# robotsorcerer/LevelSetPy

Hardware: AMD Instinct MI355X
Metric: grid-cell RK-substep updates/sec, Dubins-3D HJI 201^3 fp64 (higher is better)
Workload: dtype f64

## Files before the change

### levelsetpy_amd/csrc/hj_device.h

```cpp
#pragma once
#ifndef __HIPCC_RTC__
#include <hip/hip_runtime.h>
#endif
#include "../../include/hj_mi355x.h"

namespace hj {

template <typename T> struct Lim;
template <> struct Lim<double> { static constexpr double tiny = 1e-99; static constexpr double lowest = -1.0e300; };
template <> struct Lim<float>  { static constexpr float  tiny = 1e-30f; static constexpr float lowest = -3.0e38f; };

template <typename T> __device__ __forceinline__ T weno_eps_uncontracted(T max_d1sq) {
#pragma clang fp contract(off)
    const T a = T(1e-6) * max_d1sq;
    return a + Lim<T>::tiny;
}

template <typename T> __device__ __forceinline__ T t_abs(T x) { return x < T(0) ? -x : x; }
template <> __device__ __forceinline__ double t_abs<double>(double x) { return __builtin_fabs(x); }
template <> __device__ __forceinline__ float  t_abs<float>(float x)   { return __builtin_fabsf(x); }

__device__ __forceinline__ double max_acc(double a, double b) {
    double r;
    asm("v_max_f64 %0, %1, %2" : "=v"(r) : "v"(a), "v"(b));
// ... 268 lines not shown
        pc = T(45) * D1 + (T(-9) * D2 + D3);
        hd = T(15) * S1 + (T(-6) * S2 + (S3 + T(-20) * v[3]));
    } else if constexpr (SCHEME == HJ_WENO5) {
        const WenoLine<T> ln = weno5_line(v);
        T lq[3], rq[3];
        weno5_left_q(ln, wk, lq);
        weno5_right_q(ln, wk, rq);
        weno5_combine(ln, lq, rq, pc, hd);
    } else if constexpr ((SCHEME == HJ_ENO3 || SCHEME == HJ_ENO2) && HJ_ENO_EXACT) {
#pragma clang fp contract(off)
        DD<T> t;
        dd_tables(v, K, t);
        const T dx = K[3], dx2 = K[4], tdx2 = K[5];
        const bool sL0 = t_abs(t.D2[1]) < t_abs(t.D2[2]), sL1 = t_abs(t.D2[2]) < t_abs(t.D2[3]);
        T L, R;
        if constexpr (SCHEME == HJ_ENO2) {
            const T eL = dx * (sL0 ? t.D2[1] : t.D2[2]);
            const T eR = dx * (sL1 ? t.D2[2] : t.D2[3]);
            L = t.D1[2] + eL;
            R = t.D1[3] - eR;
        } else {
            const bool sT0 = t_abs(t.D3[0]) < t_abs(t.D3[1]), sT1 = t_abs(t.D3[1]) < t_abs(t.D3[2]);
            const bool sT2 = t_abs(t.D3[2]) < t_abs(t.D3[3]);
            const bool lRR = !sL0 && !sT1;
            const T l2 = dx * (lRR ? t.D2[2] : t.D2[1]);
            const T l3a = tdx2 * ((sL0 && sT0) ? t.D3[0] : t.D3[1]);
            const T l3b = dx2 * t.D3[2];
            const T lb = t.D1[2] + l2;
            L = lRR ? (lb - l3b) : (lb + l3a);
            const bool rRR = !sL1 && !sT2;
            const T r2 = dx * (rRR ? t.D2[3] : t.D2[2]);
            const T r3a = dx2 * ((sL1 && sT1) ? t.D3[1] : t.D3[2]);
            const T r3b = tdx2 * t.D3[3];
            const T rb = t.D1[3] - r2;
            R = rRR ? (rb + r3b) : (rb - r3a);
        }
        pc = T(0.5) * (L + R);
        hd = T(0.5) * (R - L);
    } else if constexpr (base_scheme(SCHEME) == HJ_ENO3) {
        const T u0 = v[1] - v[0], u1 = v[2] - v[1], u2 = v[3] - v[2];
        const T u3 = v[4] - v[3], u4 = v[5] - v[4], u5 = v[6] - v[5];
        const T s0 = u1 - u0, s1 = u2 - u1, s2 = u3 - u2, s3 = u4 - u3, s4 = u5 - u4;
        const T t0 = s1 - s0, t1 = s2 - s1, t2 = s3 - s2, t3 = s4 - s3;
        const bool sL0 = t_abs(s1) < t_abs(s2), sL1 = t_abs(s2) < t_abs(s3);
        const bool sT0 = t_abs(t0) < t_abs(t1), sT1 = t_abs(t1) < t_abs(t2), sT2 = t_abs(t2) < t_abs(t3);
        const T third = T(1) / T(3), sixth = T(1) / T(6);
        const T h1 = T(0.5) * s1, h2 = T(0.5) * s2, h3 = T(0.5) * s3;
        const T qL0 = third * t0 + h1, qL1 = third * t1 + h1, qL2 = h2 - sixth * t2;
        const T qR0 = -sixth * t1 - h2, qR1 = -sixth * t2 - h2, qR2 = third * t3 - h3;
        const T Lq = u2 + (sL0 ? (sT0 ? qL0 : qL1) : (sT1 ? qL1 : qL2));
        const T Rq = u3 + (sL1 ? (sT1 ? qR0 : qR1) : (sT2 ? qR1 : qR2));
        pc = Lq + Rq;
        hd = Rq - Lq;
    } else if constexpr (base_scheme(SCHEME) == HJ_ENO2) {
        const T u1 = v[2] - v[1], u2 = v[3] - v[2], u3 = v[4] - v[3], u4 = v[5] - v[4];
        const T s1 = u2 - u1, s2 = u3 - u2, s3 = u4 - u3;
        const T Lq = u2 + T(0.5) * ((t_abs(s1) < t_abs(s2)) ? s1 : s2);
        const T Rq = u3 + T(-0.5) * ((t_abs(s2) < t_abs(s3)) ? s2 : s3);
        pc = Lq + Rq;
        hd = Rq - Lq;
    } else {
        T L, R;
        upwind<SCHEME, T>(v, K, eps, L, R);
        pc = T(0.5) * (L + R);
        hd = T(0.5) * (R - L);
    }
}

#ifndef HJ_PAR_SLOTS
#define HJ_PAR_SLOTS 8
#endif
template <typename T> struct HamTables {
    const T* coord[HJ_MAX_DIM];
    const T* aux[4];
    T par[HJ_PAR_SLOTS];
    const unsigned long long* range;
    int local_mode;
};
__device__ __forceinline__ double key_value(unsigned long long k) {
    const unsigned long long b = (k & 0x8000000000000000ull) ? (k & 0x7fffffffffffffffull) : ~k;
    return __longlong_as_double((long long)b);
}

template <typename T> struct HamDubinsRel {
    static constexpr int ND = 3;
    static constexpr int ID = HJ_HAM_DUBINS_REL;
    static constexpr unsigned PLANE_DEP = 0x2;
    struct Cell { T a, b, x1, alpha0; };
    struct Plane { T x0, awx0; };
    struct Raw { T c, s, x1; };
    __device__ static __forceinline__ Raw cell_raw(const HamTables<T>& P, const int* idx) {
        return Raw{P.aux[0][idx[2]], P.aux[1][idx[2]], P.coord[1][idx[1]]};
    }
    __device__ static __forceinline__ Raw cell_raw_next(const HamTables<T>& P, const int* idx, const Raw& first) {
        return Raw{P.aux[0][idx[2]], P.aux[1][idx[2]], first.x1};
    }
    __device__ static __forceinline__ Cell cell_fin(const HamTables<T>& P, const Raw& r, const T* sc) {
#pragma clang fp contract(off)
        Cell c;
        const T a = P.par[0] - P.par[1] * r.c;
        const T b = P.par[1] * r.s;
        const T x1 = r.x1;
        c.alpha0 = sc[0] * (t_abs(a) + t_abs(P.par[2] * x1));
        c.a = sc[0] * a;
        c.b = sc[1] * b;
        c.x1 = sc[0] * x1;
        return c;
    }
    __device__ static __forceinline__ Cell cell(const HamTables<T>& P, const int* idx, const T* sc) {
        return cell_fin(P, cell_raw(P, idx), sc);
    }
    __device__ static __forceinline__ Plane plane(const HamTables<T>& P, int i0, const T* sc) {
        Plane u;
        const T x0 = P.coord[0][i0];
        u.x0 = sc[1] * x0;
        u.awx0 = sc[1] * t_abs(P.par[2] * x0);
        return u;
    }
    template <bool NP = false>
    __device__ static __forceinline__ void eval(const HamTables<T>& P, const Cell& c, const Plane& u,
                                                const T* sc, const T* q, T& H, T* alpha) {
        const T w = P.par[2];
        const T p2 = sc[2] * q[2];
        if constexpr (NP) {
#pragma clang fp contract(off)
            H = q[0] * c.a - q[1] * c.b - w * t_abs(q[0] * c.x1 - q[1] * u.x0 - p2) + w * t_abs(p2);
        } else {
            H = q[0] * c.a - q[1] * c.b - w * t_abs(q[0] * c.x1 - q[1] * u.x0 - p2) + w * t_abs(p2);
        }
        alpha[0] = c.alpha0;
        alpha[1] = t_abs(c.b) + u.awx0;
        alpha[2] = sc[2] * P.par[3];
    }
};

template <typename T> struct HamDoubleIntegrator {
    static constexpr int ND = 2;
    static constexpr int ID = HJ_HAM_DOUBLE_INTEGRATOR;
    static constexpr unsigned PLANE_DEP = 0x0;
    struct Cell { T x1, alpha0; };
    struct Plane { int unused; };
    struct Raw { T x1; };
    __device__ static __forceinline__ Raw cell_raw(const HamTables<T>& P, const int* idx) { return Raw{P.coord[1][idx[1]]}; }
    __device__ static __forceinline__ Raw cell_raw_next(const HamTables<T>& P, const int* idx, const Raw&) { return cell_raw(P, idx); }
    __device__ static __forceinline__ Cell cell_fin(const HamTables<T>&, const Raw& r, const T* sc) {
        Cell c;
        c.x1 = sc[0] * r.x1;
        c.alpha0 = sc[0] * t_abs(r.x1);
        return c;
    }
    __device__ static __forceinline__ Cell cell(const HamTables<T>& P, const int* idx, const T* sc) {
        return cell_fin(P, cell_raw(P, idx), sc);
    }
    __device__ static __forceinline__ Plane plane(const HamTables<T>&, int, const T*) { return Plane{0}; }
    template <bool NP = false>
    __device__ static __forceinline__ void eval(const HamTables<T>& P, const Cell& c, const Plane&,
                                                const T* sc, const T* q, T& H, T* alpha) {
        const T us = sc[1] * P.par[0];
        if constexpr (NP) {
#pragma clang fp contract(off)
            H = -(q[0] * c.x1 - t_abs(q[1]) * us);
        } else {
            H = -(q[0] * c.x1 - t_abs(q[1]) * us);
        }
        alpha[0] = c.alpha0;
        alpha[1] = t_abs(us);
    }
};

template <typename T> struct HamDoublePendulum {
    static constexpr int ND = 4;
    static constexpr int ID = HJ_HAM_DOUBLE_PENDULUM;
    static constexpr unsigned PLANE_DEP = 0xA;
    struct Cell { T w1, w2, s2, c2; };
    struct Plane { T s1, c1; };
    using Raw = Cell;
    struct Row { T a1, b1, c1, a3, b3, c3; };
    struct TCell { T w1s, w1q, w2s, w2q; };
    static constexpr int ROW_AXIS = 2;
    __device__ static __forceinline__ Row row(T s1, T c1, T s2, T c2, const T* sc) {
        const T G = T(9.8);
        const T sd = s2 * c1 - c2 * s1;
        const T cd = c2 * c1 + s2 * s1;
        const T den = T(2) - cd * cd;
        const T rden = T(1) / den;
        const T a = (sd * cd) * rden, c = sd * rden;
        const T b1 = (G * (s2 * cd - T(2) * s1)) * rden;
        const T b3 = (T(2) * G * (s1 * cd - s2)) * rden;
        Row r;
        r.a1 = sc[1] * a; r.b1 = sc[1] * b1; r.c1 = sc[1] * c;
        r.a3 = -(sc[3] * a); r.b3 = sc[3] * b3; r.c3 = T(-2) * (sc[3] * c);
        return r;
    }
    __device__ static __forceinline__ Row row_at(const HamTables<T>& P, int i0, int irow, const T* sc) {
        return row(P.aux[0][i0], P.aux[1][i0], P.aux[2][irow], P.aux[3][irow], sc);
    }
    __device__ static __forceinline__ TCell tcell(const Cell& c, const T* sc) {
        return TCell{sc[0] * c.w1, c.w1 * c.w1, sc[2] * c.w2, c.w2 * c.w2};
    }
    __device__ static __forceinline__ void eval_row(const HamTables<T>& P, const TCell& c, const Row& r, const T* sc, const T* q, T& H, T* alpha) {
        const T us1 = sc[1] * P.par[0], us3 = sc[3] * P.par[0];
        const T f1s = r.a1 * c.w1q + (r.c1 * c.w2q + r.b1);
        const T f3s = r.a3 * c.w2q + (r.c3 * c.w1q + r.b3);
        H = q[0] * c.w1s + (q[1] * f1s + (q[2] * c.w2s + (q[3] * f3s + (us1 * t_abs(q[1]) + us3 * t_abs(q[3])))));
        alpha[0] = t_abs(c.w1s);
        alpha[1] = t_abs(f1s) + us1;
        alpha[2] = t_abs(c.w2s);
        alpha[3] = t_abs(f3s) + us3;
    }
    __device__ static __forceinline__ Raw cell_raw(const HamTables<T>& P, const int* idx) {
        Cell c;
        c.w1 = P.coord[1][idx[1]];
        c.w2 = P.coord[3][idx[3]];
        c.s2 = P.aux[2][idx[2]];
        c.c2 = P.aux[3][idx[2]];
        return c;
    }
    __device__ static __forceinline__ Raw cell_raw_next(const HamTables<T>& P, const int* idx, const Raw& first) {
        Cell c = first;
        c.w2 = P.coord[3][idx[3]];
        return c;
    }
    __device__ static __forceinline__ Cell cell_fin(const HamTables<T>&, const Raw& r, const T*) { return r; }
    __device__ static __forceinline__ Cell cell(const HamTables<T>& P, const int* idx, const T* sc) {
        return cell_fin(P, cell_raw(P, idx), sc);
    }
    __device__ static __forceinline__ Plane plane(const HamTables<T>& P, int i0, const T*) {
        Plane u;
        u.s1 = P.aux[0][i0];
        u.c1 = P.aux[1][i0];
        return u;
    }
    template <bool NP = false>
    __device__ static __forceinline__ void eval(const HamTables<T>& P, const Cell& c, const Plane& pl,
                                                const T* sc, const T* q, T& H, T* alpha) {
        eval_row(P, tcell(c, sc), row(pl.s1, pl.c1, c.s2, c.c2, sc), sc, q, H, alpha);
    }
};
template <typename...> struct hj_void { typedef void type; };
template <typename H, typename = void> struct ham_xp { static constexpr bool value = false; };
template <typename H> struct ham_xp<H, typename hj_void<decltype(H::XPOSED)>::type> { static constexpr bool value = H::XPOSED; };
template <typename H> __host__ __device__ constexpr int ham_gaxis(int k) { return ham_xp<H>::value ? (k == 0 ? 1 : (k == 1 ? 0 : k)) : k; }

template <typename T> struct HamDubinsRelX {
    static constexpr int ND = 3;
    static constexpr int ID = HJ_HAM_DUBINS_REL;
    static constexpr bool XPOSED = true;
    static constexpr unsigned PLANE_DEP = 0x2;
    struct Cell { T a, b, x0, absa, alpha1; };
    struct Plane { T x1, awx1; };
    struct Raw { T c, s, x0; };
    __device__ static __forceinline__ Raw cell_raw(const HamTables<T>& P, const int* idx) {
        return Raw{P.aux[0][idx[2]], P.aux[1][idx[2]], P.coord[0][idx[1]]};
    }
    __device__ static __forceinline__ Raw cell_raw_next(const HamTables<T>& P, const int* idx, const Raw& first) {
        return Raw{P.aux[0][idx[2]], P.aux[1][idx[2]], first.x0};
    }
    __device__ static __forceinline__ Cell cell_fin(const HamTables<T>& P, const Raw& r, const T* sc) {
#pragma clang fp contract(off)
        Cell c;
        const T a = P.par[0] - P.par[1] * r.c;
        const T b = P.par[1] * r.s;
        c.absa = t_abs(a);
        c.a = sc[1] * a;
        c.b = sc[0] * b;
        c.x0 = sc[0] * r.x0;
        const T wx0 = P.par[2] * r.x0;
        const T awx0 = sc[0] * t_abs(wx0);
        c.alpha1 = t_abs(c.b) + awx0;
        return c;
    }
    __device__ static __forceinline__ Cell cell(const HamTables<T>& P, const int* idx, const T* sc) {
        return cell_fin(P, cell_raw(P, idx), sc);
    }
    __device__ static __forceinline__ Plane plane(const HamTables<T>& P, int im, const T* sc) {
#pragma clang fp contract(off)
        Plane u;
        const T x1 = P.coord[1][im];
        u.x1 = sc[1] * x1;
        const T wx1 = P.par[2] * x1;
        u.awx1 = t_abs(wx1);
        return u;
    }
    template <bool NP = false>
    __device__ static __forceinline__ void eval(const HamTables<T>& P, const Cell& c, const Plane& u,
                                                const T* sc, const T* q, T& H, T* alpha) {
        const T w = P.par[2];
        const T p2 = sc[2] * q[2];
        if constexpr (NP) {
#pragma clang fp contract(off)
            H = q[1] * c.a - q[0] * c.b - w * t_abs(q[1] * u.x1 - q[0] * c.x0 - p2) + w * t_abs(p2);
        } else {
            H = q[1] * c.a - q[0] * c.b - w * t_abs(q[1] * u.x1 - q[0] * c.x0 - p2) + w * t_abs(p2);
        }
        {
#pragma clang fp contract(off)
            const T sum = c.absa + u.awx1;
            alpha[1] = sc[1] * sum;
        }
        alpha[0] = c.alpha1;
        alpha[2] = sc[2] * P.par[3];
    }
};

template <typename H, typename = void> struct ham_has_rows { static constexpr bool value = false; };
template <typename H> struct ham_has_rows<H, typename hj_void<typename H::Row>::type> { static constexpr bool value = true; };

template <typename H, typename = void> struct ham_reads_range { static constexpr bool value = false; };
template <typename H> struct ham_reads_range<H, typename hj_void<decltype(H::RANGE)>::type> { static constexpr bool value = H::RANGE; };

template <bool NP, typename HAM, typename T>
__device__ __forceinline__ void lf_eval_local(const HamTables<T>& P, const typename HAM::Cell& c, const typename HAM::Plane& u,
                                              const T* sc, const T* pc, const T* hd, T& H, T* alpha) {
    constexpr int ND = HAM::ND;
    T lo[ND], hi[ND];
#pragma unroll
    for (int d = 0; d < ND; ++d) {
        const T a = sc[d] * (pc[d] - hd[d]), b = sc[d] * (pc[d] + hd[d]);
        lo[d] = a < b ? a : b;
        hi[d] = a < b ? b : a;
    }
    if (P.local_mode == 2) {
        typename HAM::Plane v = u;
#pragma unroll
        for (int d = 0; d < ND; ++d) { v.dmin[d] = lo[d]; v.dmax[d] = hi[d]; }
        HAM::template eval<NP>(P, c, v, sc, pc, H, alpha);
    } else {
#pragma unroll
        for (int i = 0; i < ND; ++i) {
            typename HAM::Plane v = u;
            v.dmin[i] = lo[i]; v.dmax[i] = hi[i];
            T Hi, ai[ND];
            HAM::template eval<NP>(P, c, v, sc, pc, Hi, ai);
            alpha[i] = ai[i];
            if (i == 0) H = Hi;
        }
    }
}

template <bool NP, typename HAM, typename T>
__device__ __forceinline__ T lf_ydot(const HamTables<T>& P, const typename HAM::Cell& c, const typename HAM::Plane& u,
                                     const T* sc, const T* pc, const T* hd, T* alpha) {
    T H;
    if constexpr (ham_reads_range<HAM>::value) {
        if (P.local_mode != 0) lf_eval_local<NP, HAM>(P, c, u, sc, pc, hd, H, alpha);
        else HAM::template eval<NP>(P, c, u, sc, pc, H, alpha);
    } else {
        HAM::template eval<NP>(P, c, u, sc, pc, H, alpha);
    }
    if constexpr (NP) {
#pragma clang fp contract(off)
        T diss = T(0);
#pragma unroll
        for (int g = 0; g < HAM::ND; ++g) diss = diss + hd[ham_gaxis<HAM>(g)] * alpha[ham_gaxis<HAM>(g)];
        return -(H - diss);
    } else {
        T diss = T(0);
#pragma unroll
        for (int g = 0; g < HAM::ND; ++g) diss += hd[ham_gaxis<HAM>(g)] * alpha[ham_gaxis<HAM>(g)];
        return -(H - diss);
    }
// ... 90 lines not shown
```

### levelsetpy_amd/csrc/hj_fusedv.h

```cpp
#pragma once
#include "hj_fused.h"

namespace hj {

#if (defined(HJ_ST_UNSAFE) || defined(HJ_ABLATE_NOSYNC) || defined(HJ_ABLATE)) && !defined(HJ_TUNE_BUILD)
#error "HJ_ST_UNSAFE / HJ_ABLATE* give wrong results: tuning builds (-DHJ_TUNE_BUILD) only"
#endif

template <typename T> struct Pair;
template <> struct Pair<double> { typedef double V __attribute__((ext_vector_type(2))); };
template <> struct Pair<float> { typedef float V __attribute__((ext_vector_type(2))); };

#ifndef HJ_PAIR_AUX_Y0
#define HJ_PAIR_AUX_Y0 0
#endif
#ifndef HJ_PAIR_AUX_OUT
#define HJ_PAIR_AUX_OUT 0
#endif
template <int AUX = 0>
__device__ __forceinline__ Pair<double>::V buf_load2(__amdgpu_buffer_rsrc_t r, unsigned off, unsigned soff, double) {
    return __builtin_bit_cast(Pair<double>::V, __builtin_amdgcn_raw_buffer_load_b128(r, off, soff, AUX));
}
template <int AUX = 0>
__device__ __forceinline__ Pair<float>::V buf_load2(__amdgpu_buffer_rsrc_t r, unsigned off, unsigned soff, float) {
    return __builtin_bit_cast(Pair<float>::V, __builtin_amdgcn_raw_buffer_load_b64(r, off, soff, AUX));
}
#ifndef HJ_ST_POST
#define HJ_ST_POST 2
#endif
#define HJ_STR2(x) #x
#define HJ_STR(x) HJ_STR2(x)
__device__ __forceinline__ void buf_store2(Pair<double>::V v, __amdgpu_buffer_rsrc_t r, unsigned off, unsigned soff) {
    using W = decltype(__builtin_amdgcn_raw_buffer_load_b128(r, off, soff, 0));
    __builtin_amdgcn_raw_buffer_store_b128(__builtin_bit_cast(W, v), r, off, soff, HJ_PAIR_AUX_OUT);
#if !defined(HJ_ST_UNSAFE)
    asm volatile("s_nop " HJ_STR(HJ_ST_POST) :: "v"(v) : "memory");
#endif
}
__device__ __forceinline__ void buf_store2(Pair<float>::V v, __amdgpu_buffer_rsrc_t r, unsigned off, unsigned soff) {
    using W = decltype(__builtin_amdgcn_raw_buffer_load_b64(r, off, soff, 0));
    __builtin_amdgcn_raw_buffer_store_b64(__builtin_bit_cast(W, v), r, off, soff, 0);
}

#define HJ_WENO_LDS_SHARE 0
#define HJ_TWO_PLANES 0
template <int K> struct IntTag { static constexpr int value = K; };
constexpr bool light_scheme_dev(int s) { return s == HJ_WENO5_ASSHIPPED || s == HJ_ENO2 || s == HJ_ENO2_FAST; }
constexpr int HJ_VPAD = 4;

template <typename T, typename HAM, int SCHEME, int NT, int R, int KH, int OCC, int MODE = 0>
__global__ __launch_bounds__(NT, OCC) void fused_pair_kernel(const T* __restrict__ y, const T* __restrict__ y0,
                                                             T* __restrict__ out, const FusedArgs<T, HAM::ND> A) {
    constexpr int ND = HAM::ND;
    constexpr int LA = ND - 1;
    constexpr int PD = 2;
    constexpr bool GEN = (MODE == 0);
    constexpr bool RNG = (MODE == 3);
    constexpr bool NP = np_order(SCHEME);
    constexpr bool XP = ham_xp<HAM>::value;
    static_assert(!XP || (ND == 3 && MODE != 3), "transposed march: 3-D substeps");
    using V = typename Pair<T>::V;
    const bool use_y0 = GEN ? (A.use_y0 != 0) : (MODE == 2);
    extern __shared__ __align__(16) unsigned char hj_smem[];
    double (*red)[ND] = reinterpret_cast<double (*)[ND]>(hj_smem);
    T* lds = reinterpret_cast<T*>(hj_smem + 512);
    static_assert((NT / 64) * ND * 8 <= 512, "reduction scratch");
    const int xb = XP ? A.xbase : 0;

    asm volatile("" ::"s"(A.nblocks), "s"(A.ntiles), "s"(A.blocks_per_xcd), "s"(A.ntile[1]), "s"(A.ntile[ND - 1]), "s"(A.E[1]),
                 "s"(A.E[ND - 1]), "s"(A.n[0]), "s"(A.n[1]), "s"(A.n[ND - 1]), "s"(A.nchunks1), "s"(A.plane_begin), "s"(A.plane_end),
                 "s"(A.plane_begin2), "s"(A.plane_end2), "s"(A.chunk), "s"(A.lpitch), "s"(A.pstride[1]), "s"(A.pstride[ND - 1]),
                 "s"(A.stride0), "s"(A.halo_lo), "s"(A.halo_hi), "s"(A.lds_nbuf), "s"(A.halo_ahead), "s"(A.timing), "s"(A.edge_blocks), "s"(A.edge_count),
                 "s"(A.nchunks_e));
    asm volatile("" ::"s"(y), "s"(y0), "s"(out), "s"(A.ham.coord[0]), "s"(A.ham.coord[1]), "s"(A.ham.coord[ND - 1]), "s"(A.ham.aux[0]),
                 "s"(A.ham.aux[1]), "s"(A.bc[1]), "s"(A.bc[ND - 1]), "s"(A.use_y0));
    const int L = logical_block(A);
    if (L < 0) return;
    const T dt_launch = launch_dt<HAM>(A);
    int chunk_id, rem;
    bool down = false;
    {
        const int paired = HJ_MAYDOWN ? 2 * A.npairs * A.ntiles : 0;
        if (L < paired) {
            int pr, r2;
            fdivmod(L, fdiv_make(2 * A.ntiles), pr, r2);
            rem = r2 >> 1;
            chunk_id = 2 * pr + (r2 & 1);
            down = (r2 & 1) == 0;
        } else {
            fdivmod(L, fdiv_make(A.ntiles), chunk_id, rem);
        }
    }
    if (A.timing && threadIdx.x == 0) {
        A.timing[4 * L + 0] = wall_clock64();
        A.timing[4 * L + 2] = (unsigned long long)(__builtin_amdgcn_s_getreg((3 << 11) | 20) & 15);
        A.timing[4 * L + 3] = (unsigned long long)chunk_id;
        A.timing[4 * (size_t)A.nblocks + 8 * (size_t)L + 4] = (unsigned long long)__builtin_amdgcn_s_getreg((31 << 11) | 4);
    }
    int org[ND], tc[ND];
    FDiv fE[ND];
    tile_coords<ND>(A, rem, tc);
#pragma unroll
    for (int d = ND - 1; d >= 1; --d) {
        org[d] = min(tc[d] * A.E[d], A.n[d] - A.E[d]);
        if (XP && d == 1) org[d] = A.xwin0 + min(tc[d] * A.E[d], (A.xwin1 - A.xwin0) - A.E[d]);
        fE[d] = fdiv_make(A.E[d]);
    }
    int p_begin, p_end;
    chunk_planes(A, chunk_id, p_begin, p_end);
    const int p_first = down ? p_end - 1 : p_begin, dirn = down ? -1 : 1;
    auto plane_at = [&](int m) { return p_first + dirn * m; };
    auto clamp_q = [&](int p) { return min(max(p, p_begin - HJ_STENCIL), p_end + HJ_STENCIL - 1); };
    auto clamp_c = [&](int p) { return min(max(p, p_begin), p_end - 1); };

    int ls[ND];
    ls[LA] = 1;
#pragma unroll
    for (int d = ND - 2; d >= 1; --d) ls[d] = (d == ND - 2) ? A.lpitch : ls[d + 1] * (A.E[d + 1] + 2 * HJ_STENCIL);
    const int lds_plane = (ND >= 3) ? ls[1] * (A.E[1] + 2 * HJ_STENCIL) : A.lpitch;
    auto pad_of = [](int d) { return d == LA ? HJ_VPAD : HJ_STENCIL; };
    int tile_cells = 1;
#pragma unroll
    for (int d = 1; d < ND; ++d) tile_cells *= A.E[d];
    const int tile_slots = tile_cells >> 1;

    const int tid = threadIdx.x;

    int own_lds[R];
    unsigned own_g[R];
    typename HAM::Cell hcell[R][2];
    typename HAM::Raw hraw[R][2];
    const bool last_real = (tid + (R - 1) * NT) < tile_slots;
    unsigned nbv[R];
#pragma unroll
    for (int r = 0; r < R; ++r) {
        int c = 2 * min(tid + r * NT, tile_slots - 1);
        int lo = 0, g = 0;
        int idx[ND];
        idx[0] = 0;
        nbv[r] = 0u;
#pragma unroll
        for (int d = ND - 1; d >= 1; --d) {
            int qd, j;
            fdivmod(c, fE[d], qd, j);
            c = qd;
            const int gi = org[d] + j;
            idx[d] = gi;
            lo += (j + pad_of(d)) * ls[d];
            g += (d == 1 ? gi - xb : gi) * A.pstride[d];
            if (j + (d == LA ? 2 : 1) < A.E[d]) nbv[r] |= 1u << d;
        }
        own_lds[r] = lo;
        own_g[r] = (unsigned)g * (unsigned)sizeof(T);
        hraw[r][0] = HAM::cell_raw(A.ham, idx);
        idx[LA] += 1;
        hraw[r][1] = HAM::cell_raw_next(A.ham, idx, hraw[r][0]);
    }

    const unsigned plane_bytes = (unsigned)(A.stride0 * (long long)sizeof(T));
    const int p_lo = p_begin - HJ_STENCIL;
    const long long xoff = XP ? (long long)xb * A.pstride[1] : 0ll;
    const unsigned xspan = XP ? A.xspan : 0u;
    const unsigned span = xspan + (unsigned)(p_end + HJ_STENCIL - p_lo) * plane_bytes;
    const __amdgpu_buffer_rsrc_t ry = make_srd(y + xoff + (long long)p_lo * A.stride0, span);
    const __amdgpu_buffer_rsrc_t ry0 = make_srd(y0 + xoff + (long long)p_lo * A.stride0, use_y0 ? span : 0u);
    const __amdgpu_buffer_rsrc_t rout = make_srd(out + xoff + (long long)p_lo * A.stride0, span);
    auto load_own = [&](int p, V* dst) {
        const bool direct = (p >= 0 || A.halo_lo) && (p < A.n[0] || A.halo_hi);
        if (direct) {
            const unsigned so = (unsigned)(p - p_lo) * plane_bytes;
#pragma unroll
            for (int r = 0; r < R; ++r) dst[r] = buf_load2(ry, own_g[r], so, T());
        } else {
            const PlaneSrc<T> s = plane_src<T, ND>(A, p);
            const __amdgpu_buffer_rsrc_t rb = make_srd(y + xoff + s.off, xspan + plane_bytes);
            if (!s.ghost) {
#pragma unroll
                for (int r = 0; r < R; ++r) dst[r] = buf_load2(rb, own_g[r], 0u, T());
            } else {
                const __amdgpu_buffer_rsrc_t ri = make_srd(y + xoff + s.off_in, xspan + plane_bytes);
#pragma unroll
                for (int r = 0; r < R; ++r) {
                    const V e = buf_load2(rb, own_g[r], 0u, T()), in = buf_load2(ri, own_g[r], 0u, T());
                    V gv;
                    gv.x = ghost_value<T>(e.x, in.x, s.km);
                    gv.y = ghost_value<T>(e.y, in.y, s.km);
                    dst[r] = gv;
                }
            }
        }
    };
    auto load_y0 = [&](int p, V* dst) {
        if (use_y0) {
            const unsigned so = (unsigned)(p - p_lo) * plane_bytes;
#pragma unroll
            for (int r = 0; r < R; ++r) dst[r] = buf_load2<HJ_PAIR_AUX_Y0>(ry0, own_g[r], so, T());
        }
    };

    T q[R][2][8];
#pragma unroll
    for (int jj = 0; jj < 7; ++jj) {
        V tmp[R];
        load_own(p_begin - 3 + jj + (down ? (p_end - 1 - p_begin) : 0), tmp);
#pragma unroll
        for (int r = 0; r < R; ++r) {
            if (down) { q[r][0][6 - jj] = tmp[r].x; q[r][1][6 - jj] = tmp[r].y; }
            else { q[r][0][jj] = tmp[r].x; q[r][1][jj] = tmp[r].y; }
        }
    }
    if (A.timing && threadIdx.x == 0) A.timing[4 * (size_t)A.nblocks + 8 * (size_t)L + 0] = wall_clock64();
    if (A.timing && threadIdx.x == 0) A.timing[4 * (size_t)A.nblocks + 8 * (size_t)L + 1] = wall_clock64();
    constexpr bool HP = (ND == 4);
    constexpr int KS = HP ? 1 : KH;
    constexpr int KP = HP ? KH - 1 : 1;
    int h_lds[KS], h_dlt[KS];
    unsigned h_src[KS];
    T h_km[KS];
    bool h_real[KS];
    int hp_lds[KP], hp_dlt[KP];
    unsigned hp_src[KP];
    T hp_km[KP];
#pragma unroll
    for (int k = 0; k < KP; ++k) { hp_lds[k] = 0; hp_dlt[k] = 0; hp_src[k] = 0; hp_km[k] = T(0); }
    if constexpr (HP) {
        int areap[ND], basep[ND + 1];
        basep[1] = 0;
        FDiv fAp[ND];
        const int half = A.E[LA] >> 1;
        const FDiv fHalf = fdiv_make(half);
#pragma unroll
        for (int d = 1; d < LA; ++d) {
            areap[d] = half;
#pragma unroll
            for (int e = 1; e < LA; ++e) if (e != d) areap[d] *= A.E[e];
            basep[d + 1] = basep[d] + 2 * HJ_STENCIL * areap[d];
            fAp[d] = fdiv_make(areap[d]);
        }
#pragma unroll
        for (int k = 0; k < KP; ++k) {
            int h = tid + k * NT;
            if (h >= basep[LA]) h = 0;
#pragma unroll
            for (int d = 1; d < LA; ++d) {
                if (h < basep[d] || h >= basep[d + 1]) continue;
                int lay, c;
                fdivmod(h - basep[d], fAp[d], lay, c);
                const int jd = (lay < HJ_STENCIL) ? (lay - HJ_STENCIL) : (A.E[d] + lay - HJ_STENCIL);
                int lo = 0, g = 0;
                {
                    int qe, j;
                    fdivmod(c, fHalf, qe, j);
                    c = qe;
                    lo += (2 * j + pad_of(LA)) * ls[LA];
                    g += (org[LA] + 2 * j) * A.pstride[LA];
// ... 39 lines not shown
            fA[d] = fdiv_make(area[d]);
        }
        const int first = HP ? base[LA] : 0;
#pragma unroll
        for (int k = 0; k < KS; ++k) {
            int h = first + tid + k * NT;
            h_real[k] = h < base[ND];
            if (!h_real[k]) h = first;
            h_lds[k] = 0; h_src[k] = 0; h_dlt[k] = 0; h_km[k] = T(0);
#pragma unroll
            for (int d = 1; d < ND; ++d) {
                if (h < base[d] || h >= base[d + 1]) continue;
                const int hh = h - base[d];
                int lay, c;
                if (d == ND - 1) {
                    c = hh / (2 * HJ_STENCIL);
                    lay = hh - c * (2 * HJ_STENCIL);
                } else {
                    fdivmod(hh, fA[d], lay, c);
                }
                const int jd = (lay < HJ_STENCIL) ? (lay - HJ_STENCIL) : (A.E[d] + lay - HJ_STENCIL);
                int lo = 0, g = 0;
#pragma unroll
                for (int e = ND - 1; e >= 1; --e) {
                    if (e == d) continue;
                    int qe, j;
                    fdivmod(c, fE[e], qe, j);
                    c = qe;
                    lo += (j + pad_of(e)) * ls[e];
                    g += (org[e] + j - (e == 1 ? xb : 0)) * A.pstride[e];
                }
                lo += (jd + pad_of(d)) * ls[d];
                int gi = org[d] + jd;
                const int nd = A.n[d];
                int dlt = 0;
                T km = T(0);
                if (gi < 0 && !(XP && d == 1 && A.xh_lo)) {
                    if (A.bc[d] == HJ_BC_PERIODIC) gi += nd;
                    else { km = T(-gi) * A.km[d]; dlt = A.pstride[d]; gi = 0; }
                } else if (gi >= nd && !(XP && d == 1 && A.xh_hi)) {
                    if (A.bc[d] == HJ_BC_PERIODIC) gi -= nd;
                    else { km = T(gi - nd + 1) * A.km[d]; dlt = -A.pstride[d]; gi = nd - 1; }
                }
                h_lds[k] = lo;
                h_src[k] = (unsigned)(g + (gi - (d == 1 ? xb : 0)) * A.pstride[d]) * (unsigned)sizeof(T);
                h_dlt[k] = dlt * (int)sizeof(T);
                h_km[k] = km;
            }
        }
    }
    bool tile_ghost = false;
#pragma unroll
    for (int d = 1; d < ND; ++d) {
        const bool below = org[d] < HJ_STENCIL && !(XP && d == 1 && A.xh_lo), above = org[d] + A.E[d] + HJ_STENCIL > A.n[d] && !(XP && d == 1 && A.xh_hi);
        tile_ghost = tile_ghost || (A.bc[d] != HJ_BC_PERIODIC && (below || above));
    }
    if (A.timing && threadIdx.x == 0) A.timing[4 * (size_t)A.nblocks + 8 * (size_t)L + 2] = wall_clock64();

    T eps[ND];
    WenoK<T> wk[ND];
#pragma unroll
    for (int d = 0; d < ND; ++d) { eps[d] = T(0); wk[d].c13 = T(0); wk[d].c4 = T(0); }
    if constexpr (SCHEME == HJ_WENO5) {
        if (A.eps_nrows > 0) fold_eps_rows<T, ND, NT>(A.eps_rows, A.eps_nrows, red, eps);
#pragma unroll
        for (int d = 0; d < ND; ++d) {
            if (A.eps_nrows <= 0) eps[d] = T(1e-6) * A.max_d1sq[ham_gaxis<HAM>(d)] + Lim<T>::tiny;
            wk[d] = weno_consts<T>(eps[d], A.K[d]);
        }
    }
    constexpr bool WCARRY = SCHEME == HJ_WENO5 && (MODE == 1 || MODE == 2);
    T wl[R][2][3];
#pragma unroll
    for (int r = 0; r < R; ++r)
#pragma unroll
        for (int c = 0; c < 2; ++c) {
            wl[r][c][0] = T(0); wl[r][c][1] = T(0); wl[r][c][2] = T(0);
            if constexpr (WCARRY) {
                if (!down) weno5_left_q(weno5_line(q[r][c]), wk[0], wl[r][c]);
            }
        }
    const bool eps_prod = SCHEME == HJ_WENO5 && A.eps_part != nullptr;
    T* const obuf = lds + A.lds_nbuf * lds_plane;
    constexpr bool WX = WCARRY && ND == 3 && HJ_WENO_LDS_SHARE;
    double dmax[ND];
    V oprev[R];
#pragma unroll
    for (int d = 0; d < ND; ++d) dmax[d] = 0.0;
#pragma unroll
    for (int r = 0; r < R; ++r) { oprev[r].x = T(0); oprev[r].y = T(0); }

    auto load_halo = [&](int p, T* dst, T* dst_in, V* dstp, V* dstp_in) {
        const unsigned so = (unsigned)(p - p_lo) * plane_bytes;
#if defined(HJ_ABLATE) && (HJ_ABLATE & 8)
        (void)so;
        return;
#endif
        if constexpr (HP) {
#pragma unroll
            for (int k = 0; k < KP; ++k) dstp[k] = buf_load2(ry, hp_src[k], so, T());
        }
#pragma unroll
        for (int k = 0; k < KS; ++k) dst[k] = buf_load(ry, h_src[k], so, T());
        if (tile_ghost) {
            if constexpr (HP) {
#pragma unroll
                for (int k = 0; k < KP; ++k) {
                    dstp_in[k].x = T(0); dstp_in[k].y = T(0);
                    if (hp_dlt[k] != 0) dstp_in[k] = buf_load2(ry, hp_src[k] + (unsigned)hp_dlt[k], so, T());
                }
            }
#pragma unroll
            for (int k = 0; k < KS; ++k) {
                dst_in[k] = T(0);
                if (h_dlt[k] != 0) dst_in[k] = buf_load(ry, h_src[k] + (unsigned)h_dlt[k], so, T());
            }
        }
    };
    auto park_halo = [&](T* bufh, const T* hv, const T* hi, const V* pv, const V* pi) {
#if !(defined(HJ_ABLATE) && (HJ_ABLATE & 16))
        if (tile_ghost) {
            if constexpr (HP) {
#pragma unroll
                for (int k = 0; k < KP; ++k) {
                    V gv;
                    gv.x = ghost_value(pv[k].x, pi[k].x, hp_km[k]);
                    gv.y = ghost_value(pv[k].y, pi[k].y, hp_km[k]);
                    *reinterpret_cast<V*>(bufh + hp_lds[k]) = gv;
                }
            }
#pragma unroll
            for (int k = 0; k < KS; ++k)
                HJ_SLOT_PRED(k) bufh[h_lds[k]] = ghost_value(hv[k], hi[k], h_km[k]);
        } else {
            if constexpr (HP) {
#pragma unroll
                for (int k = 0; k < KP; ++k) *reinterpret_cast<V*>(bufh + hp_lds[k]) = pv[k];
            }
#pragma unroll
            for (int k = 0; k < KS; ++k)
                HJ_SLOT_PRED(k) bufh[h_lds[k]] = hv[k];
        }
#else
#pragma unroll
        for (int k = 0; k < KS; ++k) asm volatile("" ::"v"(hv[k]));
        if constexpr (HP) {
#pragma unroll
            for (int k = 0; k < KP; ++k) asm volatile("" ::"v"(pv[k]));
        }
#endif
    };
    const int NB = A.lds_nbuf, AH = A.halo_ahead;
    T hal[PD][KS], hin[PD][KS];
    V halp[PD][KP], hinp[PD][KP];
#pragma unroll
    for (int s = 0; s < PD; ++s) {
#pragma unroll
        for (int k = 0; k < KS; ++k) { hal[s][k] = T(0); hin[s][k] = T(0); }
#pragma unroll
        for (int k = 0; k < KP; ++k) { halp[s][k].x = T(0); halp[s][k].y = T(0); hinp[s][k].x = T(0); hinp[s][k].y = T(0); }
    }
    constexpr int AHM = HP ? 1 : 3;
    T th[AHM][KS], ti[AHM][KS];
    V tp[AHM][KP], tq[AHM][KP];
#pragma unroll
    for (int a = 0; a < AHM; ++a) {
#pragma unroll
        for (int k = 0; k < KS; ++k) { th[a][k] = T(0); ti[a][k] = T(0); }
#pragma unroll
        for (int k = 0; k < KP; ++k) { tp[a][k].x = T(0); tp[a][k].y = T(0); tq[a][k].x = T(0); tq[a][k].y = T(0); }
        if (a < AH) load_halo(clamp_c(plane_at(a)), th[a], ti[a], tp[a], tq[a]);
    }
#pragma unroll
    for (int s = 0; s < PD; ++s) load_halo(clamp_c(plane_at(AH + s)), hal[s], hin[s], halp[s], hinp[s]);
    V own[PD][R], y0s[PD][R];
    typename HAM::Plane pls[PD];
#pragma unroll
    for (int s = 0; s < PD; ++s) {
#pragma unroll
        for (int r = 0; r < R; ++r) { own[s][r].x = T(0); own[s][r].y = T(0); }
        if (s < PD - 1) load_own(clamp_q(plane_at(4 + s)), own[s]);
    }
#pragma unroll
    for (int s = 0; s < PD; ++s) {
#pragma unroll
        for (int r = 0; r < R; ++r) { y0s[s][r].x = T(0); y0s[s][r].y = T(0); }
        const int ps = clamp_c(plane_at(s));
        load_y0(ps, y0s[s]);
        pls[s] = HAM::plane(A.ham, ps, A.sc);
    }


    if (A.timing && threadIdx.x == 0) A.timing[4 * (size_t)A.nblocks + 8 * (size_t)L + 3] = wall_clock64();
#pragma unroll
    for (int r = 0; r < R; ++r) {
        hcell[r][0] = HAM::cell_fin(A.ham, hraw[r][0], A.sc);
        hcell[r][1] = HAM::cell_fin(A.ham, hraw[r][1], A.sc);
    }
#pragma unroll
    for (int a = 0; a < AHM; ++a)
        if (a < AH) park_halo(lds + a * lds_plane, th[a], ti[a], tp[a], tq[a]);
    double amax[ND];
#pragma unroll
    for (int d = 0; d < ND; ++d) amax[d] = -1.0e300;
    constexpr bool RR = ham_reads_range<HAM>::value;
    bool local_lf = false;
    if constexpr (RR) local_lf = A.ham.local_mode != 0;
    const bool BPASS = RNG && local_lf && A.bound != nullptr;
    T lw[ND];
#pragma unroll
    for (int d = 0; d < ND; ++d) {
        lw[d] = local_lf ? (A.inv_dx[d] / A.inv_dx[0]) * (A.sc[0] / A.sc[d]) : T(0);
        if (local_lf && d > 0) amax[d] = 0.0;
    }
    auto acc_alpha = [&](const T* alpha) {
        if (RR && local_lf) {
            T ssum = T(0);
#pragma unroll
            for (int d = 0; d < ND; ++d) ssum += alpha[d] * lw[d];
            amax[0] = max_acc(amax[0], (double)ssum);
        } else {
#pragma unroll
            for (int d = 0; d < ND; ++d)
                if ((HAM::PLANE_DEP >> d) & 1u) amax[d] = max_acc(amax[d], (double)alpha[d]);
        }
    };
    T rmn[ND], rmx[ND];
#pragma unroll
    for (int d = 0; d < ND; ++d) { rmn[d] = -Lim<T>::lowest; rmx[d] = Lim<T>::lowest; }
    auto sten = [&](auto dim_tag, const T* v, T& pcv, T& hdv, bool real) {
        constexpr int d = decltype(dim_tag)::value;
        if constexpr (RNG) {
            upwind_cd<SCHEME, T>(v, A.K[d], eps[d], wk[d], pcv, hdv);
            if (real && !BPASS) range_acc(rmn[d], rmx[d], pcv, hdv);
        } else {
            upwind_cd<SCHEME, T>(v, A.K[d], eps[d], wk[d], pcv, hdv);
        }
    };

#ifdef HJ_STAMP
    unsigned long long st_acc[4] = {0, 0, 0, 0};
#endif
    int ring_c = 0;
    constexpr bool TWOB = HJ_TWO_PLANES && light_scheme_dev(SCHEME) && !HJ_MAYDOWN && ND <= 3 && MODE != 3 && !ham_xp<HAM>::value;
    int ring_of[2] = {0, 0};
    auto body = [&](auto off_tag, int m, V* own_c, V* own_n, T* hal_c, T* hin_c, V* halp_c, V* hinp_c, V* y0_c, typename HAM::Plane& pl_c) {
        constexpr int OFF = decltype(off_tag)::value;
        const int p = plane_at(m);
#ifdef HJ_STAMP
        const unsigned long long st0 = __builtin_readcyclecounter();
#endif
        T* buf = lds + ring_c * lds_plane;
        int ring_h = ring_c + AH;
        if (ring_h >= NB) ring_h -= NB;
        T* bufh = lds + ring_h * lds_plane;
        ring_c = (ring_c + 1 == NB) ? 0 : ring_c + 1;
        load_own(clamp_q(plane_at(m + 3 + PD)), own_n);
#pragma unroll
        for (int r = 0; r < R; ++r)
            if (r < R - 1 || last_real) {
                V c2;
                c2.x = q[r][0][3 + OFF];
                c2.y = q[r][1][3 + OFF];
                *reinterpret_cast<V*>(buf + own_lds[r]) = c2;
            }
        park_halo(bufh, hal_c, hin_c, halp_c, hinp_c);
#ifdef HJ_STAMP
        const unsigned long long st1 = __builtin_readcyclecounter();
#endif
#ifndef HJ_ABLATE_NOSYNC
        __syncthreads();
#endif
#ifdef HJ_STAMP
        const unsigned long long st2 = __builtin_readcyclecounter();
#endif
        const int p2 = clamp_c(plane_at(m + PD));
        load_halo(clamp_c(plane_at(m + PD + AH)), hal_c, hin_c, halp_c, hinp_c);
        const unsigned so_out = (unsigned)(p - p_lo) * plane_bytes;
        const typename HAM::Plane pl_use = pl_c;
        pl_c = HAM::plane(A.ham, p2, A.sc);
#pragma unroll
        for (int r = 0; r < R; ++r) {
            T pc[2][ND], hd[2][ND];
            const bool slot_real = r < R - 1 || last_real;
#pragma unroll
            for (int c = 0; c < 2; ++c) {
                if (down) {
                    T qg[7];
#pragma unroll
                    for (int j = 0; j < 7; ++j) qg[j] = q[r][c][6 - j + OFF];
                    sten(IntTag<0>(), qg, pc[c][0], hd[c][0], slot_real);
                } else if constexpr (WCARRY) {
                    weno5_cd_carry(q[r][c] + OFF, wk[0], wl[r][c], pc[c][0], hd[c][0]);
                } else {
                    sten(IntTag<0>(), q[r][c] + OFF, pc[c][0], hd[c][0], slot_real);
                }
            }
            const T* base = buf + own_lds[r];
#pragma unroll
            for (int d = 1; d < LA; ++d) {
                T va[7], vb[7];
#pragma unroll
                for (int j = 0; j < 7; ++j) {
                    if (j == 3) { va[j] = q[r][0][3 + OFF]; vb[j] = q[r][1][3 + OFF]; continue; }
#if defined(HJ_ABLATE) && (HJ_ABLATE & 2)
                    va[j] = q[r][0][j + OFF]; vb[j] = q[r][1][j + OFF];
#else
                    const V n2 = *reinterpret_cast<const V*>(base + (j - 3) * ls[d]);
                    va[j] = n2.x;
                    vb[j] = n2.y;
#endif
                }
                if (d == 1) { sten(IntTag<1>(), va, pc[0][1], hd[0][1], slot_real); sten(IntTag<1>(), vb, pc[1][1], hd[1][1], slot_real); }
                else { sten(IntTag<(ND > 3 ? 2 : 1)>(), va, pc[0][d], hd[0][d], slot_real); sten(IntTag<(ND > 3 ? 2 : 1)>(), vb, pc[1][d], hd[1][d], slot_real); }
            }
            {
                T w[8];
#if defined(HJ_ABLATE) && (HJ_ABLATE & 2)
                w[0] = q[r][0][0 + OFF]; w[1] = q[r][0][1 + OFF]; w[2] = q[r][0][2 + OFF]; w[5] = q[r][1][4 + OFF]; w[6] = q[r][1][5 + OFF]; w[7] = q[r][1][6 + OFF];
                w[3] = q[r][0][3 + OFF]; w[4] = q[r][1][3 + OFF];
#else
                w[0] = base[-3];
                const V l2 = *reinterpret_cast<const V*>(base - 2);
                w[1] = l2.x; w[2] = l2.y;
                w[3] = q[r][0][3 + OFF]; w[4] = q[r][1][3 + OFF];
                const V r2 = *reinterpret_cast<const V*>(base + 2);
                w[5] = r2.x; w[6] = r2.y;
                w[7] = base[4];
#endif
                if constexpr (WCARRY) {
                    weno5_cd_pair(w, wk[LA], pc[0][LA], hd[0][LA], pc[1][LA], hd[1][LA]);
                } else {
                    sten(IntTag<LA>(), w, pc[0][LA], hd[0][LA], slot_real);
                    sten(IntTag<LA>(), w + 1, pc[1][LA], hd[1][LA], slot_real);
                }
            }
            if constexpr (RNG) {
                if constexpr (RR) {
                    if (BPASS && slot_real) {
#pragma unroll
                        for (int c = 0; c < 2; ++c) {
                            T Hb, ab[ND];
                            lf_eval_local<NP, HAM>(A.ham, hcell[r][c], pl_use, A.sc, pc[c], hd[c], Hb, ab);
                            acc_alpha(ab);
                        }
                    }
                }
                continue;
            }
            V o2;
#pragma unroll
            for (int c = 0; c < 2; ++c) {
                T alpha[ND];
#if defined(HJ_ABLATE) && (HJ_ABLATE & 1)
                T ydot = pc[c][0] + hd[c][ND - 1];
#pragma unroll
                for (int d = 0; d < ND; ++d) { alpha[d] = pc[c][d]; ydot += hd[c][d]; }
#else
                T ydot = lf_ydot<NP, HAM>(A.ham, hcell[r][c], pl_use, A.sc, pc[c], hd[c], alpha);
#endif
                acc_alpha(alpha);
                if (GEN && A.do_clamp) {
                    ydot = (ydot < A.clamp_lo) ? A.clamp_lo : ydot;
                    ydot = (ydot > A.clamp_hi) ? A.clamp_hi : ydot;
                }
                const T y0v = c == 0 ? y0_c[r].x : y0_c[r].y;
                T o;
                if (GEN && A.ydot_only) o = ydot;
                else {
                    o = rk_stage_out<NP>(A.stage, A.ca, A.cb, dt_launch, y0v, q[r][c][3 + OFF], ydot);
                    if (GEN && A.post_op) o = post_step(A.post_op, o, use_y0 ? y0v : q[r][c][3 + OFF]);
                }
                if (c == 0) o2.x = o; else o2.y = o;
            }
            if (r < R - 1 || last_real) buf_store2(o2, rout, own_g[r], so_out);
            if constexpr (SCHEME == HJ_WENO5) {
                if (eps_prod) {
                    T* ob = obuf + ((p - p_begin) & 1) * lds_plane;
                    dmax[LA] = fmax(dmax[LA], (double)t_abs(o2.y - o2.x));
                    if (p > p_begin) {
                        dmax[0] = fmax(dmax[0], fmax((double)t_abs(o2.x - oprev[r].x), (double)t_abs(o2.y - oprev[r].y)));
                        const T* op = obuf + ((p - p_begin - 1) & 1) * lds_plane + own_lds[r];
#pragma unroll
                        for (int d = 1; d < LA; ++d)
                            if ((nbv[r] >> d) & 1u) {
                                const V n2 = *reinterpret_cast<const V*>(op + ls[d]);
                                dmax[d] = fmax(dmax[d], fmax((double)t_abs(n2.x - oprev[r].x), (double)t_abs(n2.y - oprev[r].y)));
                            }
                        if ((nbv[r] >> LA) & 1u) dmax[LA] = fmax(dmax[LA], (double)t_abs(op[2] - oprev[r].y));
                    }
                    *reinterpret_cast<V*>(ob + own_lds[r]) = o2;
                    oprev[r] = o2;
                }
            }
        }
#ifdef HJ_STAMP
        const unsigned long long st3 = __builtin_readcyclecounter();
#endif
        load_y0(p2, y0_c);
#pragma unroll
        for (int r = 0; r < R; ++r) {
            if constexpr (OFF == 0) {
                q[r][0][7] = own_c[r].x;
                q[r][1][7] = own_c[r].y;
            } else {
#pragma unroll
                for (int j = 0; j < 6; ++j) { q[r][0][j] = q[r][0][j + 2]; q[r][1][j] = q[r][1][j + 2]; }
                q[r][0][6] = own_c[r].x;
                q[r][1][6] = own_c[r].y;
            }
        }
#ifdef HJ_STAMP
        {
            const unsigned long long st4 = __builtin_readcyclecounter();
            st_acc[0] += st1 - st0; st_acc[1] += st2 - st1; st_acc[2] += st3 - st2; st_acc[3] += st4 - st3;
        }
#endif
    };

    if (A.timing && tid == 0) A.timing[4 * (size_t)A.nblocks + 8 * (size_t)L + 5] = wall_clock64();
    const int nplanes = p_end - p_begin;
    for (int m = 0; m < nplanes; m += PD) {
        body(IntTag<0>(), m, own[0], own[1], hal[0], hin[0], halp[0], hinp[0], y0s[0], pls[0]);
        if (m + 1 < nplanes) body(IntTag<1>(), m + 1, own[1], own[0], hal[1], hin[1], halp[1], hinp[1], y0s[1], pls[1]);
        if (A.timing && tid == 0 && m == 0) A.timing[4 * (size_t)A.nblocks + 8 * (size_t)L + 7] = wall_clock64();
    }
    if (A.timing && tid == 0) A.timing[4 * (size_t)A.nblocks + 8 * (size_t)L + 6] = wall_clock64();

    if constexpr (RNG) {
        if (!BPASS) {
            publish_range<ND, NT>(A.range_keys, red, rmn, rmx, A.sc);
            return;
        }
    }
    if constexpr (SCHEME == HJ_WENO5) {
        if (eps_prod) {
            __syncthreads();
            if (p_end > p_begin) {
#pragma unroll
                for (int r = 0; r < R; ++r) {
                    const T* op = obuf + ((p_end - 1 - p_begin) & 1) * lds_plane + own_lds[r];
#pragma unroll
                    for (int d = 1; d < LA; ++d)
                        if ((nbv[r] >> d) & 1u) {
                            const V n2 = *reinterpret_cast<const V*>(op + ls[d]);
                            dmax[d] = fmax(dmax[d], fmax((double)t_abs(n2.x - oprev[r].x), (double)t_abs(n2.y - oprev[r].y)));
                        }
                    if ((nbv[r] >> LA) & 1u) dmax[LA] = fmax(dmax[LA], (double)t_abs(op[2] - oprev[r].y));
                }
            }
            store_eps_part<ND, NT>(A.eps_part + (size_t)L * HJ_MAX_DIM, red, dmax);
        }
    }
    if (A.bound) {
        {
            T pz[ND], Hz, az[ND];
    #pragma unroll
            for (int d = 0; d < ND; ++d) pz[d] = T(0);
    #pragma unroll
            for (int r = 0; r < R; ++r)
    #pragma unroll
                for (int c = 0; c < 2; ++c) {
                    HAM::eval(A.ham, hcell[r][c], pls[0], A.sc, pz, Hz, az);
    #pragma unroll
                    for (int d = 0; d < ND; ++d)
                        if (!((HAM::PLANE_DEP >> d) & 1u)) amax[d] = fmax(amax[d], (double)az[d]);
                }
        }

        const int lane = tid & 63, wv = tid >> 6;
    #pragma unroll
        for (int d = 0; d < ND; ++d) {
            const double m = wave_max(amax[d]) / (double)A.sc[d];
            if (lane == 0) red[wv][d] = m;
        }
        __syncthreads();
        if (tid < ND) {
            double m = red[0][tid];
            for (int w = 1; w < NT / 64; ++w) m = fmax(m, red[w][tid]);
            if (m > -1.0e299) key_max(A.bound + (XP ? (tid == 0 ? 1 : (tid == 1 ? 0 : tid)) : tid), m);
        }
    }
    publish_gate(A, chunk_id);
    if (A.timing && tid == 0) A.timing[4 * L + 1] = wall_clock64();
#ifdef HJ_STAMP
    if (A.timing && tid == 0)
        for (int k = 0; k < 4; ++k) A.timing[4 * (size_t)A.nblocks + 8 * (size_t)L + k] = st_acc[k];
#endif
}

}
```

Measured before the change: 224.9 billion.

## Split plane loop into branch-free interior path and boundary tail; load plane tables via constant address space

The plane-sweep loop is split into an interior phase and a general tail. In the interior phase, loads of the next plane go straight to the buffer without boundary/halo checks, and stores skip the last-real predicate. Per-plane coordinate and trig table reads are cast to the constant address space (4) so the compiler can use scalar loads. A volatile v_mov copy is inserted on interior register rotation, and a waitcnt is issued before the interior loop. This trims branch and predicate overhead in the hot loop at the cost of more code, plus a risk if the interior bounds are computed wrongly.

```diff
diff --git a/levelsetpy_amd/csrc/hj_device.h b/levelsetpy_amd/csrc/hj_device.h
--- a/levelsetpy_amd/csrc/hj_device.h
+++ b/levelsetpy_amd/csrc/hj_device.h
@@ -374,6 +374,11 @@
     return __longlong_as_double((long long)b);
 }
 
+template <typename T> __device__ __forceinline__ T table_at(const T* tab, int i) {
+    typedef const T __attribute__((address_space(4))) * CPtr;
+    return ((CPtr)tab)[i];
+}
+
 template <typename T> struct HamDubinsRel {
     static constexpr int ND = 3;
     static constexpr int ID = HJ_HAM_DUBINS_REL;
@@ -404,7 +409,7 @@
     }
     __device__ static __forceinline__ Plane plane(const HamTables<T>& P, int i0, const T* sc) {
         Plane u;
-        const T x0 = P.coord[0][i0];
+        const T x0 = table_at(P.coord[0], i0);
         u.x0 = sc[1] * x0;
         u.awx0 = sc[1] * t_abs(P.par[2] * x0);
         return u;
@@ -519,8 +524,8 @@
     }
     __device__ static __forceinline__ Plane plane(const HamTables<T>& P, int i0, const T*) {
         Plane u;
-        u.s1 = P.aux[0][i0];
-        u.c1 = P.aux[1][i0];
+        u.s1 = table_at(P.aux[0], i0);
+        u.c1 = table_at(P.aux[1], i0);
         return u;
     }
     template <bool NP = false>
@@ -568,7 +573,7 @@
     __device__ static __forceinline__ Plane plane(const HamTables<T>& P, int im, const T* sc) {
 #pragma clang fp contract(off)
         Plane u;
-        const T x1 = P.coord[1][im];
+        const T x1 = table_at(P.coord[1], im);
         u.x1 = sc[1] * x1;
         const T wx1 = P.par[2] * x1;
         u.awx1 = t_abs(wx1);
diff --git a/levelsetpy_amd/csrc/hj_fusedv.h b/levelsetpy_amd/csrc/hj_fusedv.h
--- a/levelsetpy_amd/csrc/hj_fusedv.h
+++ b/levelsetpy_amd/csrc/hj_fusedv.h
@@ -42,10 +42,9 @@
     __builtin_amdgcn_raw_buffer_store_b64(__builtin_bit_cast(W, v), r, off, soff, 0);
 }
 
-#define HJ_WENO_LDS_SHARE 0
-#define HJ_TWO_PLANES 0
+__device__ __forceinline__ double queue_copy(double v) { double r; asm volatile("v_mov_b64 %0, %1" : "=v"(r) : "v"(v)); return r; }
+__device__ __forceinline__ float queue_copy(float v) { float r; asm volatile("v_mov_b32 %0, %1" : "=v"(r) : "v"(v)); return r; }
 template <int K> struct IntTag { static constexpr int value = K; };
-constexpr bool light_scheme_dev(int s) { return s == HJ_WENO5_ASSHIPPED || s == HJ_ENO2 || s == HJ_ENO2_FAST; }
 constexpr int HJ_VPAD = 4;
 
 template <typename T, typename HAM, int SCHEME, int NT, int R, int KH, int OCC, int MODE = 0>
@@ -165,12 +164,15 @@
     const __amdgpu_buffer_rsrc_t ry = make_srd(y + xoff + (long long)p_lo * A.stride0, span);
     const __amdgpu_buffer_rsrc_t ry0 = make_srd(y0 + xoff + (long long)p_lo * A.stride0, use_y0 ? span : 0u);
     const __amdgpu_buffer_rsrc_t rout = make_srd(out + xoff + (long long)p_lo * A.stride0, span);
+    auto load_own_direct = [&](int p, V* dst) {
+        const unsigned so = (unsigned)(p - p_lo) * plane_bytes;
+#pragma unroll
+        for (int r = 0; r < R; ++r) dst[r] = buf_load2(ry, own_g[r], so, T());
+    };
     auto load_own = [&](int p, V* dst) {
         const bool direct = (p >= 0 || A.halo_lo) && (p < A.n[0] || A.halo_hi);
         if (direct) {
-            const unsigned so = (unsigned)(p - p_lo) * plane_bytes;
-#pragma unroll
-            for (int r = 0; r < R; ++r) dst[r] = buf_load2(ry, own_g[r], so, T());
+            load_own_direct(p, dst);
         } else {
             const PlaneSrc<T> s = plane_src<T, ND>(A, p);
             const __amdgpu_buffer_rsrc_t rb = make_srd(y + xoff + s.off, xspan + plane_bytes);
@@ -376,7 +378,6 @@
         }
     const bool eps_prod = SCHEME == HJ_WENO5 && A.eps_part != nullptr;
     T* const obuf = lds + A.lds_nbuf * lds_plane;
-    constexpr bool WX = WCARRY && ND == 3 && HJ_WENO_LDS_SHARE;
     double dmax[ND];
     V oprev[R];
 #pragma unroll
@@ -536,10 +537,9 @@
     unsigned long long st_acc[4] = {0, 0, 0, 0};
 #endif
     int ring_c = 0;
-    constexpr bool TWOB = HJ_TWO_PLANES && light_scheme_dev(SCHEME) && !HJ_MAYDOWN && ND <= 3 && MODE != 3 && !ham_xp<HAM>::value;
-    int ring_of[2] = {0, 0};
-    auto body = [&](auto off_tag, int m, V* own_c, V* own_n, T* hal_c, T* hin_c, V* halp_c, V* hinp_c, V* y0_c, typename HAM::Plane& pl_c) {
+    auto body = [&](auto off_tag, auto int_tag, int m, V* own_c, V* own_n, T* hal_c, T* hin_c, V* halp_c, V* hinp_c, V* y0_c, typename HAM::Plane& pl_c) {
         constexpr int OFF = decltype(off_tag)::value;
+        constexpr bool INTERIOR = decltype(int_tag)::value != 0;
         const int p = plane_at(m);
 #ifdef HJ_STAMP
         const unsigned long long st0 = __builtin_readcyclecounter();
@@ -549,7 +549,8 @@
         if (ring_h >= NB) ring_h -= NB;
         T* bufh = lds + ring_h * lds_plane;
         ring_c = (ring_c + 1 == NB) ? 0 : ring_c + 1;
-        load_own(clamp_q(plane_at(m + 3 + PD)), own_n);
+        if constexpr (INTERIOR) load_own_direct(plane_at(m + 3 + PD), own_n);
+        else load_own(clamp_q(plane_at(m + 3 + PD)), own_n);
 #pragma unroll
         for (int r = 0; r < R; ++r)
             if (r < R - 1 || last_real) {
@@ -667,7 +668,7 @@
                 }
                 if (c == 0) o2.x = o; else o2.y = o;
             }
-            if (r < R - 1 || last_real) buf_store2(o2, rout, own_g[r], so_out);
+            if (INTERIOR || r < R - 1 || last_real) buf_store2(o2, rout, own_g[r], so_out);
             if constexpr (SCHEME == HJ_WENO5) {
                 if (eps_prod) {
                     T* ob = obuf + ((p - p_begin) & 1) * lds_plane;
@@ -694,14 +695,15 @@
         load_y0(p2, y0_c);
 #pragma unroll
         for (int r = 0; r < R; ++r) {
+            const T oc0 = INTERIOR ? queue_copy(own_c[r].x) : own_c[r].x, oc1 = INTERIOR ? queue_copy(own_c[r].y) : own_c[r].y;
             if constexpr (OFF == 0) {
-                q[r][0][7] = own_c[r].x;
-                q[r][1][7] = own_c[r].y;
+                q[r][0][7] = oc0;
+                q[r][1][7] = oc1;
             } else {
 #pragma unroll
                 for (int j = 0; j < 6; ++j) { q[r][0][j] = q[r][0][j + 2]; q[r][1][j] = q[r][1][j + 2]; }
-                q[r][0][6] = own_c[r].x;
-                q[r][1][6] = own_c[r].y;
+                q[r][0][6] = oc0;
+                q[r][1][6] = oc1;
             }
         }
 #ifdef HJ_STAMP
@@ -714,9 +716,24 @@
 
     if (A.timing && tid == 0) A.timing[4 * (size_t)A.nblocks + 8 * (size_t)L + 5] = wall_clock64();
     const int nplanes = p_end - p_begin;
-    for (int m = 0; m < nplanes; m += PD) {
-        body(IntTag<0>(), m, own[0], own[1], hal[0], hin[0], halp[0], hinp[0], y0s[0], pls[0]);
-        if (m + 1 < nplanes) body(IntTag<1>(), m + 1, own[1], own[0], hal[1], hin[1], halp[1], hinp[1], y0s[1], pls[1]);
+    int m = 0;
+    {
+        const int q_lo = max(p_begin - HJ_STENCIL, A.halo_lo ? -(1 << 30) : 0), q_hi = min(p_end + HJ_STENCIL - 1, A.halo_hi ? (1 << 30) : A.n[0] - 1);
+        const int p5 = plane_at(3 + PD);
+        const int j_max = (p5 >= q_lo && p5 <= q_hi) ? (down ? p_end - 1 - q_lo : q_hi - p_begin) : -1;
+        if (m + 4 + PD <= j_max) {
+            __builtin_amdgcn_s_waitcnt(0x0F70);
+            do {
+                body(IntTag<0>(), IntTag<1>(), m, own[0], own[1], hal[0], hin[0], halp[0], hinp[0], y0s[0], pls[0]);
+                body(IntTag<1>(), IntTag<1>(), m + 1, own[1], own[0], hal[1], hin[1], halp[1], hinp[1], y0s[1], pls[1]);
+                if (A.timing && tid == 0 && m == 0) A.timing[4 * (size_t)A.nblocks + 8 * (size_t)L + 7] = wall_clock64();
+                m += PD;
+            } while (m + 4 + PD <= j_max);
+        }
+    }
+    for (; m < nplanes; m += PD) {
+        body(IntTag<0>(), IntTag<0>(), m, own[0], own[1], hal[0], hin[0], halp[0], hinp[0], y0s[0], pls[0]);
+        if (m + 1 < nplanes) body(IntTag<1>(), IntTag<0>(), m + 1, own[1], own[0], hal[1], hin[1], halp[1], hinp[1], y0s[1], pls[1]);
         if (A.timing && tid == 0 && m == 0) A.timing[4 * (size_t)A.nblocks + 8 * (size_t)L + 7] = wall_clock64();
     }
     if (A.timing && tid == 0) A.timing[4 * (size_t)A.nblocks + 8 * (size_t)L + 6] = wall_clock64();
```

Result: no change. 224.2 billion (-0.3%).
